# Helkafen/find-tfbs

Measured on AMD Instinct MI355X. Metric: haplotype-windows scored/sec, higher is better.
Workload: dtype fp4xfp6->f32 bound + int32 exact

## Files before the change

### find-tfbs_amd/csrc/ctx_assembly.hip

```cpp
#include "ctx.hpp"

using namespace tfbs;

AsmArgs tfbs::asm_args(tfbs_ctx *ctx, const Batch &B, int mode) {
    AsmArgs a{};
    a.haps = ctx->img.haps.p;
    a.druns = ctx->img.druns.p;
    a.regions = ctx->img.regions.p;
    a.hap_reuse = ctx->img.hap_reuse.p;
    a.region_asm = ctx->img.region_asm.p;
    a.inner = ctx->img.inner.p;
    a.mmeta = ctx->tabs.m_meta.p;
    a.slot_mfma = ctx->tabs.slot_mfma.p;
    a.any_dense = (!ctx->plan.fast_tiles.empty() || !ctx->plan.gen_tiles.empty() || !ctx->plan.di_tiles.empty()) ? 1 : 0;
    a.n_slots = B.n_slots;
    a.hpb = ctx->knobs.mfma_hpb;
    a.hitl = ctx->scan.hitl.p;
    a.hitn = ctx->scan.hitn.p;
    a.cand_cap = ctx->scan.scan_hit_cap;
    a.mfma = ctx->plan.m_supers.empty() ? 0 : 1;
    a.ref_hits = ctx->scan.ref_hits.p;
    a.ref_count = ctx->scan.ref_count.p;
    a.spill_sorted = ctx->scan.spill_sorted.p;
    a.spill_off = ctx->scan.spill_boff.p;
// ... 142 lines not shown
    uint64_t t_lo = UINT64_MAX, t_hi = 0;
    double busy = 0;
    for (uint32_t r = 0; r < nr; r++) {
        const uint64_t *p = &h[(size_t)r * kKfProfWords];
        if (!p[6]) continue;
        t_lo = std::min(t_lo, p[0]);
        t_hi = std::max(t_hi, p[6]);
        busy += (double)(p[6] - p[0]);
    }
    {
        std::vector<std::pair<std::pair<uint64_t, uint64_t>, uint32_t>> ev;
        for (uint32_t r = 0; r < nr; r++)
            if (h[(size_t)r * kKfProfWords + 6]) ev.push_back({{h[(size_t)r * kKfProfWords + 14], h[(size_t)r * kKfProfWords]}, r});
        std::sort(ev.begin(), ev.end());
        double gap = 0, late = 0, early_end = 0;
        uint32_t n_gap = 0, n_groups = 0;
        for (size_t i = 0; i < ev.size(); i++) {
            const uint64_t *p = &h[(size_t)ev[i].second * kKfProfWords];
            const bool first = i == 0 || ev[i - 1].first.first != ev[i].first.first;
            const bool last = i + 1 == ev.size() || ev[i + 1].first.first != ev[i].first.first;
            if (first) {
                n_groups++;
                late += (double)(p[0] - t_lo);
            } else {
                gap += (double)(p[0] - h[(size_t)ev[i - 1].second * kKfProfWords + 6]);
                n_gap++;
            }
            if (last) early_end += (double)(t_hi - p[6]);
        }
        if (n_groups)
            fprintf(stderr, "[kf prof] %u workgroups: mean gap between a workgroup's regions %.1f us (%u gaps), first "
                            "region start after the kernel's first %.1f us, last end before the kernel's last %.1f us\n",
                    n_groups, n_gap ? gap / n_gap / 100.0 : 0.0, n_gap, late / n_groups / 100.0, early_end / n_groups / 100.0);
    }
    uint32_t early = 0;
    for (uint32_t r = 0; r < nr; r++)
        if (h[(size_t)r * kKfProfWords + 6] && h[(size_t)r * kKfProfWords] < t_lo + 1000) early++;
    if (t_hi > t_lo)
        fprintf(stderr, "[kf prof] span %.1f us (first region start to last end, 100 MHz ticks), region-time %.1f us: "
                        "%.0f regions in flight on average; %u regions started in the first 10 us\n",
                (t_hi - t_lo) / 100.0, busy / 100.0, busy / (double)(t_hi - t_lo), early);
    const double d = n ? n : 1;
    fprintf(stderr,
            "[kf prof] front ticks/region: region record + reference hit list (round 1) %.0f, descriptors + hitn + "
            "first runs + meta (round 2) %.0f, hitn scan %.0f, runs staged %.0f, reference hits + barrier %.0f; in front of "
            "a region, ticket atomic to order entry %.0f\n",
            fr[0] / d, fr[1] / d, fr[2] / d, fr[3] / d, fr[4] / d, tkt / d);
    fprintf(stderr,
            "[kf prof] regions %u of %u ticks/region: descr+hitn %.0f refs %.0f dirty %.0f lists %.0f keys %.0f "
            "chunks %.0f (of which var-list atomics %.0f) (max total %.0f); per region: U %.1f entries %.1f dirty-refs %.1f corrections %.1f rows "
            "%.1f chunks %.2f in-LDS %.2f refs %.1f\n",
            n, nr, ph[0] / d, ph[1] / d, ph[2] / d, ph[3] / d, ph[4] / d, ph[5] / d, at / d, mx, sz[0] / d, sz[1] / d,
            sz[2] / d, sz[3] / d, sz[4] / d, sz[5] / d, sz[6] / d, sz[7] / d);
    return TFBS_OK;
}

int tfbs::assembly_wait(tfbs_ctx *ctx, Batch &B) {
    for (int round = 0; ctx->asmb.asm_state == 1; round++) {
        if (round == 8) return tfbs::fail(TFBS_E_NOMEM, "scan / key lists still full after 8 reruns");
        HIP_TRY(hipEventSynchronize(ctx->asmb.asm_ev));
        const uint32_t nspill = ctx->asmb.asm_host[kCtrOver], ncand = ctx->asmb.asm_host[kCtrOver + 1];
        const uint64_t *vt = reinterpret_cast<const uint64_t *>(ctx->asmb.asm_host.p + kCtrVarTot);
        const uint64_t nk = vt[0], nc = vt[1];
        if (ctx->knobs.debug_over && ctx->asmb.asm_host[kCtrRedoN]) {
            std::vector<uint32_t> redo(ctx->asmb.asm_host[kCtrRedoN]);
            HIP_TRY(hipMemcpy(redo.data(), ctx->asmb.asm_redo.p, redo.size() * 4, hipMemcpyDeviceToHost));
            uint64_t su = 0, sr = 0;
            uint32_t mu = 0, mi = 0;
            for (uint32_t r : redo) {
                const DevRegion &rg = B.regions[r];
                su += rg.hap_count;
                mu = std::max(mu, rg.hap_count);
                mi = std::max(mi, rg.n_inner);
                for (uint32_t l = 0; l < rg.hap_count; l++) sr += B.haps[rg.hap_begin + l].n_druns;
            }
            const uint32_t *why = ctx->asmb.asm_host.p + kCtrWhy;
            fprintf(stderr, "tfbs assembly: %zu regions left to key_asm: mean haplotypes %.1f (max %u), max inner %u, "
                            "mean diff runs %.1f; reasons: shape %u lists %u runs %u refs %u arena(cor) %u arena(cnt) %u\n",
                    redo.size(), (double)su / redo.size(), mu, mi, (double)sr / redo.size(), why[0], why[1], why[2],
                    why[3], why[4], why[5]);
        }
        if (ctx->knobs.debug_over)
            fprintf(stderr, "tfbs assembly: spill %u/%u candidates %u/%u left to key_asm %u arena %u/%u varying keys "
                            "%llu/%u counts %llu/%llu\n", nspill, ctx->scan.spill_cap, ncand, ctx->scan.cand_over_cap,
                    ctx->asmb.asm_host[kCtrRedoN], ctx->asmb.asm_host[kCtrCorUsed], ctx->asmb.cor_cap,
                    (unsigned long long)nk, ctx->asmb.var_keys_cap, (unsigned long long)nc,
                    (unsigned long long)ctx->asmb.var_cap);
        int rc;
        const bool need_post = !ctx->asmb.stages.post && (nspill || ncand);
        const bool need_wide = !ctx->asmb.stages.wide && ctx->asmb.asm_host[kCtrNeedWide], need_left = !ctx->asmb.stages.leftover && ctx->asmb.asm_host[kCtrRedoN];
        if (need_post || need_wide || need_left) {
            ctx->asmb.asm_full = true;
            ctx->asmb.asm_reruns++;
            ctx->asmb.asm_reruns_post += need_post ? 1 : 0;
            ctx->asmb.asm_post_rerun = need_post;
            ctx->asmb.asm_reruns_wide += need_wide ? 1 : 0;
            ctx->asmb.asm_reruns_left += need_left ? 1 : 0;
            rc = enqueue_assembly(ctx, B, true);
            ctx->asmb.asm_full = false;
            if (rc) return rc;
            continue;
        }
        if (ctx->asmb.asm_host[kCtrCorUsed] > ctx->asmb.cor_cap)
            ctx->asmb.cor_cap = (uint32_t)std::min<uint64_t>((uint64_t)ctx->asmb.asm_host[kCtrCorUsed] * 5 / 4, 1u << 30);
        if (nspill > ctx->scan.spill_cap || ncand > ctx->scan.cand_over_cap) {
            grow_cap(ctx->scan.spill_cap, ncand > ctx->scan.cand_over_cap ? 2 * std::max(nspill, 1024u) : nspill, UINT32_MAX / 4);
// ... 300 lines not shown
```

### find-tfbs_amd/csrc/key_kernels.hip

```cpp
#include <hip/hip_runtime.h>

#include <mutex>

#include <algorithm>
#include <cstdio>
#include <cstdlib>
#include <string>
#include <type_traits>

#include "keys.hpp"

namespace tfbs {
namespace {

constexpr int kAsmBlock = 256;
constexpr uint32_t kAsmWaves = kAsmBlock / 64;
constexpr uint32_t kAsmCounters = 6144;
constexpr uint32_t kAsmHaps = 1024;

constexpr uint32_t kAsmRuns = 2048;
constexpr uint32_t kAsmHits = 2048;
constexpr uint32_t kAsmRefs = 256;
constexpr uint32_t kAsmKeyWords = 2048;
constexpr uint32_t kAsmKeyWin = 32 * kAsmKeyWords;
// ... 391 lines not shown
using KfTyped = std::true_type;
using KfAny = std::false_type;
typedef uint32_t kf_u32x2 __attribute__((ext_vector_type(2)));
__device__ __forceinline__ uint32_t ld_global(const uint32_t *p) {
    return *(const __attribute__((address_space(1))) uint32_t *)p;
}
__device__ __forceinline__ uint2 ld_global(const uint2 *p) {
    const kf_u32x2 v = *(const __attribute__((address_space(1))) kf_u32x2 *)p;
    return make_uint2(v.x, v.y);
}
__device__ __forceinline__ void st_global(uint32_t *p, uint32_t v) {
    *(__attribute__((address_space(1))) uint32_t *)p = v;
}

__device__ __forceinline__ void arrived(uint32_t &x) { asm volatile("" : "+v"(x)); }

template <class Put>
__device__ __forceinline__ void wave_push(Put &&put, uint32_t *n, uint32_t cap, bool want, uint32_t v) {
    const uint64_t m = __ballot(want);
    if (!m) return;
    const uint32_t lane = threadIdx.x & 63, leader = (uint32_t)__builtin_ctzll(m);
    uint32_t base = 0;
    if (lane == leader) base = atomicAdd(n, (uint32_t)__popcll(m));
    base = (uint32_t)__shfl((int)base, (int)leader);
    if (want) {
        const uint32_t at = base + __builtin_amdgcn_mbcnt_hi((uint32_t)(m >> 32), __builtin_amdgcn_mbcnt_lo((uint32_t)m, 0));
        if (at < cap) put(at, v);
    }
}

template <uint32_t kFWaves>
__device__ __forceinline__ uint32_t block_excl_scan(uint32_t v, uint32_t *s_w, uint32_t &total) {
    const uint32_t lane = threadIdx.x & 63, wave = threadIdx.x >> 6;
    uint32_t x = v;
#pragma unroll
    for (int o = 1; o < 64; o <<= 1) {
        const uint32_t y = (uint32_t)__shfl_up((int)x, o);
        if (lane >= (uint32_t)o) x += y;
    }
    if (lane == 63) s_w[wave] = x;
    __syncthreads();
    uint32_t pre = 0, tot = 0;
#pragma unroll
    for (uint32_t w = 0; w < kFWaves; w++) {
        const uint32_t t = s_w[w];
        pre += w < wave ? t : 0u;
        tot += t;
    }
    __syncthreads();
    total = tot;
    return pre + x - v;
}

#ifndef TFBS_KF_WAVES
#define TFBS_KF_WAVES 1
#endif
template <class C>
__global__ __launch_bounds__(C::kBlock) __attribute__((amdgpu_waves_per_eu(C::kBlock == 1024 ? 1 : TFBS_KF_WAVES)))
void key_fast_kernel(AsmArgs A, uint32_t first, uint32_t count, uint32_t which) {
    constexpr int kFBlock = C::kBlock;
    constexpr uint32_t kFWaves = C::kWaves, kFHapLds = C::kHapLds, kFCor = C::kCor, kFRefs = C::kRefs,
                       kFCnt = C::kCnt, kFRuns = C::kRuns, kFRows = C::kRows, kFLists = C::kLists;
    constexpr uint32_t kPerW = kFKeyWords >= (uint32_t)kFBlock ? kFKeyWords / kFBlock : 1u;
    __shared__ uint32_t s_cor[kFCor];
    __shared__ uint4 s_ref[kFRefs];
    __shared__ uint32_t s_hap[kFHapLds];
    __shared__ uint32_t s_cnt[kFCnt];
    uint2 *const s_run = reinterpret_cast<uint2 *>(s_cnt);
    __shared__ uint32_t s_bits[kFKeyWords], s_rbase[kFKeyWords];
    __shared__ uint32_t s_rkey[kFRows], s_rr[kFRows];
    __shared__ uint32_t s_loff[kFLists + 1], s_lidx[kFLists];
    __shared__ uint32_t s_w[kFWaves];
    __shared__ uint32_t s_ncor, s_nref, s_nvar, s_arena, s_ndirty;
    __shared__ unsigned long long s_vbase, s_obase;
    const uint32_t tid = threadIdx.x, lane = tid & 63, wave = tid >> 6;
    auto process = [&](const uint32_t r, const uint32_t by_ticket, const uint64_t t_ticket) {
    auto stamp = [&](uint32_t k, uint64_t v) {
        if (A.prof && tid == 0) A.prof[kKfProfWords * (size_t)r + k] = v;
    };
    stamp(0, wall_clock64());
    stamp(20, t_ticket);
    uint32_t ft = tid;
    arrived(ft);
    const uint32_t *const none = reinterpret_cast<const uint32_t *>(A.regions + r);
    auto have = [&](bool c, const auto *p) { return c ? p : reinterpret_cast<decltype(p)>(none); };
    const bool spills = A.spill_count != nullptr;
    uint32_t n_rc = ld_global(have(A.mfma, A.ref_count + r));
    const uint2 rh = ld_global(have(A.mfma, reinterpret_cast<const uint2 *>(A.ref_hits) + (size_t)r * kRefPerRegion + (ft & 63u)));
    uint32_t rh_g = rh.x, rh_i = rh.y;
    uint32_t sp_n = ld_global(have(spills, A.spill_count));
    uint32_t sp_c = ld_global(have(spills, A.spill_cnt + r));
    uint32_t sp_o = ld_global(have(spills, A.spill_off + r));
    DevRegion rg = A.regions[r];
    uint4 ra = A.region_asm[r];
    arrived(n_rc), arrived(rh_g), arrived(rh_i), arrived(sp_n), arrived(sp_c), arrived(sp_o);
    arrived(rg.hap_count), arrived(ra.x);
    if (!spills) sp_n = 0;
    stamp(16, wall_clock64());
    const uint32_t U = rg.hap_count, n_inner = rg.n_inner, K = A.n_slots * n_inner;
    const uint64_t ko = (uint64_t)rg.inner_off * A.n_slots;
    uint32_t pw = TFBS_PATH_FAST | (kFBlock == 1024 ? TFBS_PATH_BIG : 0u) | by_ticket;
    auto trace = [&](uint32_t w) {
        if (A.path && tid == 0) A.path[r] = w;
    };
    if (U == 0 || K == 0) {
        trace(pw);
        for (uint32_t j = tid; j < K; j += kFBlock) {
            A.key_first[ko + j] = 0;
            A.key_flags[ko + j] = 0;
        }
        return;
    }
    auto give_up = [&](uint32_t why) {
        if (tid == 0) {
            A.redo[atomicAdd(A.redo_n, 1u)] = r;
            if (A.why) atomicAdd(A.why + why, 1u);
        }
        trace(pw | TFBS_PATH_GIVEUP | (why << TFBS_PATH_WHY_SHIFT));
    };
    if (U > (kFMaxU < A.fast_max_u ? kFMaxU : A.fast_max_u) || K > 32 * kFKeyWords || n_inner > 32) return give_up(0);
    const uint32_t hb = rg.hap_begin;
    const bool refs_on = A.mfma && rg.ref_hap != UINT32_MAX;
    const uint32_t run0 = (uint32_t)__builtin_amdgcn_readfirstlane((int)ra.x);
    const uint32_t nruns = (uint32_t)__builtin_amdgcn_readfirstlane((int)ra.y);
    const uint32_t lmax = (uint32_t)__builtin_amdgcn_readfirstlane((int)ra.z);
    if (tid == 0) s_ncor = s_nref = s_ndirty = 0;
    const uint32_t g_lo = hb / A.hpb, g_hi = (hb + U - 1) / A.hpb;
    const uint32_t nl = A.mfma ? (g_hi + 1 - g_lo) * kMBlockWaves : 0u;
    auto list_idx = [&](uint32_t t) -> uint32_t { return g_lo * kMBlockWaves + t; };
    const bool lists_staged = nl <= kFLists;
    if (!lists_staged) pw |= TFBS_PATH_LISTS_SLICED;
    if (nruns >= 65536) return give_up(2);
    if (nruns > kFRuns) pw |= TFBS_PATH_RUNS_L2;
    constexpr uint32_t kHapQ = kFHapLds / kFBlock;
// ... 36 lines not shown
    stamp(1, wall_clock64());
    auto hap_info = [&](uint32_t l) -> uint32_t {
        if (l < kFHapLds) return s_hap[l];
        return ld_global(A.hap_reuse + hb + l);
    };
    auto run_at = [&](auto typed, uint32_t k) -> uint2 {
        if constexpr (decltype(typed)::value) {
            return s_run[k];
        } else {
            if (runs_lds) return s_run[k];
            return ld_global(druns + k);
        }
    };
    if (runs_lds) {
        if (tid < nruns) s_run[tid] = make_uint2(run_a, run_b);
        for (uint32_t k = tid + kFBlock; k < nruns; k += kFBlock) s_run[k] = ld_global(druns + k);
    }
    stamp(18, wall_clock64());
    const uint2 sp = sp_n && sp_c ? make_uint2(sp_o, sp_o + sp_c) : make_uint2(0, 0);
    if (refs_on) {
        if (tid < n_list) {
            const uint32_t at = atomicAdd(&s_nref, 1u);
            if (at < kFRefs) s_ref[at] = make_ref_loaded(A, rg, m_len, m_depth, m_slot, rh_i);
        }
        for (uint32_t e = sp.x + tid; e < sp.y; e += kFBlock) {
            const uint32_t *q = A.spill_sorted + 3 * (size_t)e;
            if (q[0] >> 31) {
                const uint32_t at = atomicAdd(&s_nref, 1u);
                if (at < kFRefs) s_ref[at] = make_ref(A, rg, q[1], q[2]);
            }
        }
    }
    __syncthreads();
    const uint32_t nref = s_nref;
    stamp(19, wall_clock64());
    if (nref > kFRefs) return give_up(3);
    const bool pairwise = (uint64_t)U * nref <= 65536;
    if (!pairwise) pw |= TFBS_PATH_WALK;
    if (!pairwise) {
        uint4 mine = make_uint4(0, 0, 0, 0);
        uint32_t rank = 0;
        if (tid < nref) {
            mine = s_ref[tid];
            for (uint32_t j = 0; j < nref; j++) {
                const uint32_t w = s_ref[j].y;
                rank += (w < mine.y || (w == mine.y && j < tid)) ? 1u : 0u;
            }
        }
        __syncthreads();
        if (tid < nref) s_ref[rank] = mine;
        __syncthreads();
    }
    stamp(2, wall_clock64());
    auto dirty_masks = [&](auto typed, auto &&f) {
        for (uint32_t l0 = wave * 64; l0 < U; l0 += kFBlock) {
            const uint32_t l = l0 + lane;
            const uint32_t x = l < U ? hap_info(l) : kFNone;
            const uint32_t k0 = x == kFNone ? 0u : x & 0xFFFFu, k1 = x == kFNone ? 0u : k0 + (x >> 16);
            for (uint32_t p0 = 0; p0 < nref; p0 += 64) {
                const uint32_t np = min(64u, nref - p0);
                uint32_t rw = 0, re = 0;
                if (lane < np) {
                    const uint4 q = s_ref[p0 + lane];
                    rw = q.y;
                    re = q.y + (q.z & 0xFFFFu) - 1;
                }
                uint64_t m = 0;
                for (uint32_t i = 0; __ballot(i < k1 - k0) != 0; i++) {
                    uint2 ab = make_uint2(0xFFFFFFFFu, 0u);
                    if (i < k1 - k0) ab = run_at(typed, k0 + i);
                    for (uint32_t p = 0; p < np; p++) {
                        const uint32_t w = (uint32_t)__builtin_amdgcn_readlane((int)rw, (int)p);
                        const uint32_t e = (uint32_t)__builtin_amdgcn_readlane((int)re, (int)p);
                        if (ab.x <= e && ab.y >= w) m |= 1ull << p;
                    }
                }
                f(l, p0, m);
            }
        }
    };
    auto dirty_walk = [&](auto typed, auto &&f) {
        for (uint32_t l = tid; l < U; l += kFBlock) {
            const uint32_t x = hap_info(l);
            if (x == kFNone) continue;
            const uint32_t k0 = x & 0xFFFFu, k1 = k0 + (x >> 16);
            uint32_t p = 0;
            for (uint32_t k = k0; k < k1 && p < nref; k++) {
                const uint2 ab = run_at(typed, k);
                const uint32_t a = ab.x, b = ab.y;
                const uint32_t lo = a >= kMChunkCols * kMMaxChunks - 1 ? a - (kMChunkCols * kMMaxChunks - 1) : 0u;
                while (p < nref && s_ref[p].y < lo) p++;
                for (; p < nref && s_ref[p].y <= b; p++) {
                    const uint4 q = s_ref[p];
                    bool dirty = false;
                    for (uint32_t k2 = k0; k2 < k1 && !dirty; k2++) {
                        const uint2 r2 = run_at(typed, k2);
                        dirty = run_meets(r2.x, r2.y, q.y, q.z & 0xFFFFu);
                    }
                    if (dirty) f(l, q);
                }
            }
        }
    };
    auto slots = [&](uint32_t c, uint32_t *ctr) -> uint32_t {
        if (!__ballot(c > 1)) {
            const uint64_t m = __ballot(c != 0);
            if (!m) return 0;
            const uint32_t leader = (uint32_t)__builtin_ctzll(m);
            uint32_t base = 0;
            if (lane == leader) base = atomicAdd(ctr, (uint32_t)__popcll(m));
            return (uint32_t)__shfl((int)base, (int)leader) +
                   __builtin_amdgcn_mbcnt_hi((uint32_t)(m >> 32), __builtin_amdgcn_mbcnt_lo((uint32_t)m, 0));
        }
        uint32_t x = c;
#pragma unroll
        for (int o = 1; o < 64; o <<= 1) {
            const uint32_t y = (uint32_t)__shfl_up((int)x, o);
            if (lane >= (uint32_t)o) x += y;
        }
        const uint32_t tot = (uint32_t)__shfl((int)x, 63);
        uint32_t base = 0;
        if (lane == 0 && tot) base = atomicAdd(ctr, tot);
        return (uint32_t)__shfl((int)base, 0) + x - c;
    };
    auto list_mask = [&](uint32_t l, uint32_t p0, uint64_t m, uint32_t *ctr, auto &&put) -> uint32_t {
        uint32_t c = 0;
        for (uint64_t b = m; b; b &= b - 1) c += __popc(s_ref[p0 + (uint32_t)__builtin_ctzll(b)].w);
        uint32_t at = slots(c, ctr);
        for (uint64_t b = m; b; b &= b - 1) {
            const uint4 q = s_ref[p0 + (uint32_t)__builtin_ctzll(b)];
            for (uint32_t w = q.w; w; w &= w - 1, at++) put(at, cor_entry(q.x + __builtin_ctz(w), l, 1));
        }
        return c;
    };
    const uint32_t rpl = nref <= 1 ? 1u : nref >= 64 ? 64u : 1u << (32 - __clz(nref - 1));
    const uint32_t hpw = 64 / rpl, n_p = (nref + rpl - 1) / rpl;
    const bool stepbits = pairwise && (U + kFWaves * hpw - 1) / (kFWaves * hpw) * n_p <= 64;
    uint32_t nd = 0;
    if (nref) {
        auto count_and_list = [&](auto typed) {
            if (pairwise)
                dirty_masks(typed, [&](uint32_t l, uint32_t p0, uint64_t m) {
                    nd += list_mask(l, p0, m, &s_ndirty, [&](uint32_t at, uint32_t v) {
                        if (at < kFCor) s_cor[kFCor - 1 - at] = v;
                    });
                });
            else
                dirty_walk(typed, [&](uint32_t, const uint4 &q) { nd += __popc(q.w); });
        };
        if (runs_lds) count_and_list(KfTyped{});
        else count_and_list(KfAny{});
    }
    uint32_t nD = 0;
    (void)block_excl_scan<kFWaves>(nd, s_w, nD);
    const bool dirty_listed = pairwise && nD <= kFCor;
    const uint32_t need = n_ent + (sp.y - sp.x) + nD;
    const bool in_lds = need <= (kFCor < A.cor_lds ? kFCor : A.cor_lds);
    pw |= (stepbits ? TFBS_PATH_STEPBITS : 0u) | (dirty_listed ? TFBS_PATH_DIRTY_LISTED : 0u) |
          (in_lds ? 0u : TFBS_PATH_COR_ARENA);
    if (tid == 0) {
        s_arena = kFNone;
        if (!in_lds) {
            const uint32_t at = atomicAdd(A.cor_used, need);
            if (at <= A.cor_cap && need <= A.cor_cap - at) s_arena = at;
            if (dirty_listed) s_ncor = nD;
        }
    }
    __syncthreads();
    if (!in_lds && s_arena == kFNone) return give_up(4);
    stamp(3, wall_clock64());
    uint32_t *const cor_g = A.cor_arena + (in_lds ? 0u : s_arena);
    auto cor_ld = [&](auto typed, uint32_t e) -> uint32_t {
        if constexpr (decltype(typed)::value) {
            return s_cor[e];
        } else {
            if (in_lds) return s_cor[e];
            return ld_global(cor_g + e);
        }
    };
    auto cor_st = [&](auto typed, uint32_t e, uint32_t v) {
        if constexpr (decltype(typed)::value) {
            s_cor[e] = v;
        } else {
            if (in_lds) s_cor[e] = v;
            else st_global(cor_g + e, v);
        }
    };
    if (!in_lds && dirty_listed)
        for (uint32_t e = tid; e < nD; e += kFBlock) st_global(cor_g + e, s_cor[kFCor - 1 - e]);
    const uint32_t nw = (K + 31) / 32;
    uint32_t nA = 0, nB = 0, ncor = 0, T = 0;
    auto lists_and_rows = [&](auto typed) {
    auto put = [&](uint32_t at, uint32_t v) { cor_st(typed, at, v); };
    const uint2 *hitl = reinterpret_cast<const uint2 *>(A.hitl);
    for (uint32_t l0 = 0; l0 < nl; l0 += kFLists) {
        const uint32_t nlc = min(kFLists, nl - l0);
        uint32_t tot = n_ent;
        if (!lists_staged) {
            uint32_t lc = 0;
            if (tid < nlc) {
                const uint32_t idx = list_idx(l0 + tid);
                lc = A.hitn[idx];
                s_lidx[tid] = idx;
            }
            const uint32_t off = block_excl_scan<kFWaves>(lc, s_w, tot);
            if (tid < nlc) s_loff[tid] = off;
            if (tid == 0) s_loff[nlc] = tot;
            __syncthreads();
        }
        for (uint32_t e0 = 0; e0 < tot; e0 += kFBlock * kFBatch) {
            uint2 h[kFBatch];
#pragma unroll
            for (uint32_t q = 0; q < kFBatch; q++) {
                const uint32_t e = e0 + q * kFBlock + tid;
                h[q] = make_uint2(hb + U, 0);
                if (e < tot) {
                    uint32_t lo = 0, hi = nlc - 1;
                    while (lo < hi) {
                        const uint32_t mid = (lo + hi + 1) / 2;
                        if (s_loff[mid] <= e) lo = mid;
                        else hi = mid - 1;
                    }
                    const uint32_t idx = s_lidx[lo];
                    h[q] = hitl[(size_t)(idx / kMBlockWaves) * A.cand_cap +
                                (size_t)(idx % kMBlockWaves) * (A.cand_cap / kMBlockWaves) + (e - s_loff[lo])];
                }
            }
#pragma unroll
            for (uint32_t q = 0; q < kFBatch; q++)
                wave_push(put, &s_ncor, need, h[q].x - hb < U, cor_entry(h[q].y, h[q].x - hb, 0));
        }
        __syncthreads();
    }
    for (uint32_t e0 = sp.x; e0 < sp.y; e0 += kFBlock) {
        const uint32_t e = e0 + tid;
        bool want = false;
        uint32_t v = 0;
        if (e < sp.y) {
            const uint32_t *q = A.spill_sorted + 3 * (size_t)e;
            want = !(q[0] >> 31) && q[1] - hb < U;
            v = cor_entry(q[2], q[1] - hb, 0);
        }
        wave_push(put, &s_ncor, need, want, v);
    }
    if (!dirty_listed && nref) {
        auto put_in = [&](uint32_t at, uint32_t v) {
            if (at < need) cor_st(typed, at, v);
        };
        if (pairwise)
            dirty_masks(typed, [&](uint32_t l, uint32_t p0, uint64_t m) { (void)list_mask(l, p0, m, &s_ncor, put_in); });
        else
            dirty_walk(typed, [&](uint32_t l, const uint4 &q) {
                uint32_t at = atomicAdd(&s_ncor, (uint32_t)__popc(q.w));
                for (uint32_t m = q.w; m; m &= m - 1, at++) put_in(at, cor_entry(q.x + __builtin_ctz(m), l, 1));
            });
    }
    for (uint32_t w = tid; w < nw; w += kFBlock) s_bits[w] = 0;
    __syncthreads();
    stamp(4, wall_clock64());
    nA = s_ncor, nB = in_lds && dirty_listed ? nD : 0u, ncor = nA + nB;
    for (uint32_t e = tid; e < nA; e += kFBlock) {
        const uint32_t c = cor_ld(typed, e);
        if (!cor_neg(c)) atomicOr(&s_bits[cor_key(c) >> 5], 1u << (cor_key(c) & 31u));
    }
    if (tid < nref)
        for (uint32_t m = s_ref[tid].w; m; m &= m - 1) {
            const uint32_t key = s_ref[tid].x + __builtin_ctz(m);
            atomicOr(&s_bits[key >> 5], 1u << (key & 31u));
        }
    if (A.any_dense)
        for (uint32_t j = tid; j < K; j += kFBlock)
            if (!A.slot_mfma[j / n_inner]) atomicOr(&s_bits[j >> 5], 1u << (j & 31u));
    __syncthreads();
    {
        constexpr uint32_t per = kPerW;
        uint32_t mine = 0;
#pragma unroll
        for (uint32_t q = 0; q < per; q++) {
            const uint32_t w = tid * per + q;
            if (w < nw) mine += __popc(s_bits[w]);
        }
        uint32_t run = block_excl_scan<kFWaves>(mine, s_w, T);
#pragma unroll
        for (uint32_t q = 0; q < per; q++) {
            const uint32_t w = tid * per + q;
            if (w < nw) {
                s_rbase[w] = run;
                run += __popc(s_bits[w]);
            }
        }
    }
    };
    if (in_lds && runs_lds) lists_and_rows(KfTyped{});
    else lists_and_rows(KfAny{});
    stamp(5, wall_clock64());
    auto row_of = [&](uint32_t j) { return s_rbase[j >> 5] + __popc(s_bits[j >> 5] & ((1u << (j & 31)) - 1u)); };
    const bool half = 4 * (lmax + 64) < 65536 && A.cor_lds != 0;
    uint32_t rows_per = min((half ? 2 : 1) * kFCnt / U, kFRows);
    uint16_t *const cnt16 = reinterpret_cast<uint16_t *>(s_cnt);
    bool h16 = half, cnt_arena = false;
    uint32_t *cnt_g = A.cor_arena;
    if ((T + rows_per - 1) / rows_per > 32 || A.cor_lds == 0) {
        h16 = false;
        cnt_arena = true;
        pw |= TFBS_PATH_CNT_ARENA;
        rows_per = min(T, kFRows);
        if (tid == 0) {
            s_arena = kFNone;
            const uint32_t want = rows_per * U, at = atomicAdd(A.cor_used, want);
            if (at <= A.cor_cap && want <= A.cor_cap - at) s_arena = at;
        }
        __syncthreads();
        if (s_arena == kFNone) return give_up(5);
        cnt_g = A.cor_arena + s_arena;
    }
    pw |= (h16 ? 0u : TFBS_PATH_U32) | (U > kFHapLds ? TFBS_PATH_HAP_GLOBAL : 0u);
    for (uint32_t j = tid; j < K; j += kFBlock)
        if (!((s_bits[j >> 5] >> (j & 31)) & 1u)) {
            A.key_first[ko + j] = 0;
            A.key_flags[ko + j] = 0;
        }
    const uint64_t dense_base = A.dense_base ? A.haps[hb].count_off : 0;
    uint64_t t_atomics = 0;
    auto chunks = [&](auto typed) {
    constexpr bool kTyped = decltype(typed)::value;
    auto cor_top = [&](uint32_t e) -> uint32_t { return kFCor - nB + (e - nA); };
    auto cor_at = [&](uint32_t e) -> uint32_t {
        if constexpr (kTyped) return s_cor[e < nA ? e : cor_top(e)];
        else return e < nA ? cor_ld(typed, e) : s_cor[cor_top(e)];
    };
    auto cnt_set = [&](uint32_t x, uint32_t v) {
        if (kTyped || h16) cnt16[x] = (uint16_t)v;
        else if (cnt_arena) st_global(cnt_g + x, v);
        else s_cnt[x] = v;
    };
    auto cnt_add = [&](uint32_t x, uint32_t d) {
        if (kTyped || h16) atomicAdd(&s_cnt[x >> 1], d << (16 * (x & 1u)));
        else if (cnt_arena) atomicAdd(&cnt_g[x], d);
        else atomicAdd(&s_cnt[x], d);
    };
    auto count_at = [&](uint32_t x) -> uint32_t {
        if (kTyped || h16) return (uint32_t)cnt16[x];
        if (cnt_arena) return ld_global(cnt_g + x);
        return s_cnt[x];
    };
    for (uint32_t e = tid; e < ncor; e += kFBlock) {
        const uint32_t c = cor_at(e), v = (row_of(cor_key(c)) << 12) | (c & 4095u);
        if (e < nA) cor_st(typed, e, v);
        else s_cor[cor_top(e)] = v;
    }
    uint32_t dedup_bits = 0;
    for (uint32_t i = 0, l = lane; l < U; i++, l += 64)
        if (hap_info(l) != kFNone) dedup_bits |= 1u << i;
    for (uint32_t t0 = 0; t0 < T; t0 += rows_per) {
        const uint32_t nrow = min(rows_per, T - t0);
        __syncthreads();
        if (tid == 0) s_nvar = 0;
        {
            constexpr uint32_t per = kPerW;
#pragma unroll
            for (uint32_t q = 0; q < per; q++) {
                const uint32_t w = tid * per + q;
                if (w >= nw) continue;
                uint32_t t = s_rbase[w], b = s_bits[w];
                if (t >= t0 + nrow || t + __popc(b) <= t0) continue;
                for (; b; b &= b - 1, t++)
                    if (t - t0 < nrow) s_rkey[t - t0] = 32 * w + __builtin_ctz(b);
            }
        }
        for (uint32_t rr = tid; rr < nrow; rr += kFBlock) s_rr[rr] = 0;
        __syncthreads();
        if (tid < nref)
            for (uint32_t m = s_ref[tid].w; m; m &= m - 1) {
                const uint32_t t = row_of(s_ref[tid].x + __builtin_ctz(m)) - t0;
                if (t < nrow) atomicAdd(&s_rr[t], 1u);
            }
        __syncthreads();
        for (uint32_t rr = wave; rr < nrow; rr += kFWaves) {
            const uint32_t j = s_rkey[rr], R = s_rr[rr];
            const bool dense = A.any_dense && !A.slot_mfma[j / n_inner];
            for (uint32_t i = 0, l = lane; l < U; i++, l += 64) {
                const uint32_t v = dense ? A.counts[dense_base + (uint64_t)j * rg.count_stride + l]
                                         : ((dedup_bits >> i) & 1u ? R : 0u);
                cnt_set(rr * U + l, v);
            }
        }
        __syncthreads();
        for (uint32_t e = tid; e < ncor; e += kFBlock) {
            const uint32_t c = cor_at(e);
            const uint32_t t = cor_key(c) - t0;
            if (t < nrow) cnt_add(t * U + cor_hap(c), cor_neg(c) ? 0xFFFFFFFFu : 1u);
        }
        __syncthreads();
        for (uint32_t rr = wave; rr < nrow; rr += kFWaves) {
            const uint32_t c0 = count_at(rr * U);
            uint32_t any = 0, diff = 0;
            for (uint32_t l = lane; l < U; l += 64) {
                const uint32_t c = count_at(rr * U + l);
                any |= c;
                diff |= c ^ c0;
            }
            const bool a = __ballot(any != 0) != 0, v = __ballot(diff != 0) != 0;
            if (lane == 0) {
                const uint32_t j = s_rkey[rr];
                A.key_first[ko + j] = c0;
                A.key_flags[ko + j] = (uint8_t)((a ? KEY_ANY : 0) | (v ? KEY_VARIES : 0));
                s_rr[rr] = v ? atomicAdd(&s_nvar, 1u) : kFNone;
            }
        }
        __syncthreads();
        const uint64_t ta = A.prof ? wall_clock64() : 0;
        if (tid == 0 && s_nvar) {
            s_vbase = atomicAdd(A.var_tot, (unsigned long long)s_nvar);
            s_obase = atomicAdd(A.var_tot + 1, (unsigned long long)s_nvar * U);
        }
        __syncthreads();
        if (A.prof) t_atomics += wall_clock64() - ta;
        for (uint32_t rr = wave; rr < nrow; rr += kFWaves) {
            const uint32_t slot = s_rr[rr];
            if (slot == kFNone) continue;
            const uint64_t vi = s_vbase + slot, off = s_obase + (uint64_t)slot * U;
            if (vi >= A.var_keys_cap || off + U > A.var_cap) continue;
            if (lane == 0) A.var_keys[vi] = DevVarKey{r, s_rkey[rr], off};
            for (uint32_t l = lane; l < U; l += 64) A.var_counts[off + l] = count_at(rr * U + l);
        }
    }
    };
    if (in_lds && h16) chunks(KfTyped{});
    else chunks(KfAny{});
    stamp(6, wall_clock64());
    stamp(7, t_atomics);
    stamp(8, U);
    stamp(9, n_ent);
    stamp(10, nD);
    stamp(11, ncor);
    stamp(12, T);
    stamp(13, (T + rows_per - 1) / rows_per);
    stamp(14, blockIdx.x | (which << 24));
    stamp(15, nref);
    trace(pw);
    };
    __shared__ uint32_t s_tk;
    const bool tickets = A.persist && gridDim.x < count;
    uint32_t i = blockIdx.x;
    while (i < count) {
        uint32_t tk = 0;
        uint64_t t_ticket = A.prof ? wall_clock64() : 0;
        if (tickets && tid == 0) tk = gridDim.x + atomicAdd(A.next + which, 1u);
        const uint32_t r = A.order ? A.order[first + i] : first + i;
        if (A.prof) {
            asm volatile("" ::"v"(r));
            t_ticket = wall_clock64() - t_ticket;
        }
        process(r, i == blockIdx.x ? 0u : (uint32_t)TFBS_PATH_TICKET, t_ticket);
        if (!tickets) break;
        if (tid == 0) s_tk = tk;
        __syncthreads();
        i = s_tk;
        __syncthreads();
    }
    if (A.report_fast && blockIdx.x == 0 && tid < 2) A.report[tid] = A.report_src ? A.report_src[tid] : 0u;
}

__global__ __launch_bounds__(256) void spill_hist_kernel(const uint32_t *__restrict__ over, uint32_t cap,
                                                          const uint32_t *__restrict__ spill, uint32_t *__restrict__ bcnt) {
    const uint32_t n = min(over[0], cap);
    for (uint32_t e = blockIdx.x * 256 + threadIdx.x; e < n; e += gridDim.x * 256)
        atomicAdd(&bcnt[spill[3 * (size_t)e] & 0x7FFFFFFFu], 1u);
}

__global__ __launch_bounds__(1024) void spill_scan_kernel(const uint32_t *__restrict__ over, uint32_t *__restrict__ bcnt,
                                                          uint32_t n, uint32_t *__restrict__ boff) {
    __shared__ uint32_t s[1024];
    if (over[0] == 0) return;
    uint32_t carry = 0;
    for (uint32_t b0 = 0; b0 < n; b0 += 1024) {
        const uint32_t i = b0 + threadIdx.x;
        const uint32_t v = i < n ? bcnt[i] : 0;
        s[threadIdx.x] = v;
        __syncthreads();
        for (uint32_t o = 1; o < 1024; o <<= 1) {
            const uint32_t t = threadIdx.x >= o ? s[threadIdx.x - o] : 0;
            __syncthreads();
            s[threadIdx.x] += t;
// ... 422 lines not shown
```

### find-tfbs_amd/csrc/keys.hpp

```cpp
#pragma once

#include <hip/hip_runtime.h>

#include <algorithm>
#include <cstddef>
#include <cstdint>

#include "batch.hpp"
#include "scan.hpp"

namespace tfbs {

struct AsmArgs {
    const DevHap *haps;
    const uint32_t *druns;
    const DevRegion *regions;
    const uint32_t *hap_reuse;
    const uint4 *region_asm;
    const int32_t *inner;
    const int32_t *mmeta;
    const uint8_t *slot_mfma;
    uint32_t any_dense;
    uint32_t n_slots;
    uint32_t hpb;
    const uint32_t *hitl, *hitn;
    uint32_t cand_cap;
    uint32_t mfma;
    const uint32_t *ref_hits, *ref_count;
    const uint32_t *spill_sorted, *spill_off, *spill_cnt;
    const uint32_t *spill_count;
    uint32_t spill_cap;
    uint32_t *counts;
    uint32_t dense_base;
    uint32_t *scratch;
    int mode;
    uint32_t *key_first;
    uint8_t *key_flags;
    DevVarKey *var_keys;
    uint32_t var_keys_cap;
    uint32_t *var_counts;
    uint64_t var_cap;
    unsigned long long *var_tot;
    uint32_t *redo, *redo_n;
    uint32_t fast_max_u;
    uint32_t *cor_arena;
    uint32_t cor_cap;
    uint32_t *cor_used;
    uint32_t cor_lds;
    uint32_t *why;
    const uint32_t *report_src;
    uint32_t *report;
    uint32_t report_fast;
    const uint32_t *order;
    uint32_t persist;
    uint32_t *next;
    uint64_t *prof;
    uint32_t *path;
    uint32_t grid_cap;
};

constexpr uint32_t kKfProfWords = 24;

enum AsmCtr : uint32_t {
    kCtrOver = 0,
    kCtrRedoN = 2,
    kCtrCorUsed = 3,
    kCtrVarTot = 4,
    kCtrWhy = 8,
    kCtrNext = 16,
    kCtrWgDone = 18,
    kCtrNeedWide = 20,
    kCtrPostDone = 21,
    kAsmCtrWords = 24,
};
inline size_t asm_bucket_words(uint32_t nr) { return 2 * ((size_t)std::max<uint32_t>(1, nr) + 1); }

int launch_key_asm(const AsmArgs &a, uint32_t n_regions, hipStream_t stream);
int launch_key_fast(const AsmArgs &a, uint32_t n_regions, uint32_t n_big, hipStream_t stream, hipStream_t side,
                    hipEvent_t fork, hipEvent_t join, bool leftover = true);
uint32_t key_fast_big_u();
int launch_asm_report(const uint32_t *over, uint32_t *ctr, hipStream_t stream);
uint32_t key_asm_lds_counters();
int launch_spill_buckets(const uint32_t *over, uint32_t cap, const uint32_t *spill, uint32_t n_regions, uint32_t *bcnt,
                         uint32_t *boff, uint32_t *sorted, hipStream_t stream, bool bcnt_zeroed = false);
int launch_pair_table(const uint64_t *rows, uint32_t n_regions, uint32_t n_samples, uint32_t *pab, uint32_t *pcnt,
                      uint32_t *pair_n, uint16_t *pidx, hipStream_t stream);
int launch_memb_fill(const uint32_t *meta, const uint32_t *ids, const uint16_t *loc, uint32_t n_rows, uint32_t Hp,
                     uint16_t *memb, hipStream_t stream);
int launch_key_encode(const uint32_t *var_counts, const DevVarKey *keys, uint32_t n_keys, const uint32_t *pab,
                      const uint32_t *pcnt, const uint32_t *pair_n, const uint16_t *pidx, uint32_t region0,
                      uint32_t n_samples, EncHdr *hdr, uint32_t *vals, uint32_t *hist, uint8_t *codes,
                      hipStream_t stream);
int launch_val_compact(const uint32_t *vals, const uint32_t *hist, uint32_t n_keys, const uint32_t *off, uint32_t *ov,
                       uint32_t *oh, hipStream_t stream);
int launch_code_compact(const uint8_t *codes, uint32_t n_keys, uint32_t n_samples, const uint64_t *off, uint8_t *dst,
                        hipStream_t stream);

}
```

Baseline: 331700 billion.

## Restructure key_fast dirty-hit listing and chunk loop; raise waves per EU

Replaces the per-hap dirty mask loop with a grouped readlane comparison that splits references across spare waves and lists hits with one atomic per block of 64 haps. For non-1024-thread blocks, rewrites the chunk loop so each wave owns rows with one row per lane: row keys are built once when they fit, reference counts come from ballots, classification and variable-key slot allocation are done per lane, and the var_tot atomics are issued by the first two threads. It also raises the default waves-per-EU hint from 1 to 4 and adds optional fine-grained profiling compiled in only under a macro. The changes trade simpler code and register headroom for more parallel work per region, and they add an extra barrier.

```diff
diff --git a/find-tfbs_amd/csrc/ctx_assembly.hip b/find-tfbs_amd/csrc/ctx_assembly.hip
--- a/find-tfbs_amd/csrc/ctx_assembly.hip
+++ b/find-tfbs_amd/csrc/ctx_assembly.hip
@@ -218,6 +218,18 @@
             "%.1f chunks %.2f in-LDS %.2f refs %.1f\n",
             n, nr, ph[0] / d, ph[1] / d, ph[2] / d, ph[3] / d, ph[4] / d, ph[5] / d, at / d, mx, sz[0] / d, sz[1] / d,
             sz[2] / d, sz[3] / d, sz[4] / d, sz[5] / d, sz[6] / d, sz[7] / d);
+    double fine[kKfProfFineN] = {}, fine_sum = 0;
+    for (uint32_t r = 0; r < nr; r++) {
+        const uint64_t *p = &h[(size_t)r * kKfProfWords];
+        if (!p[6]) continue;
+        for (uint32_t k = 0; k < kKfProfFineN; k++) fine[k] += (double)p[kKfProfFine + k], fine_sum += (double)p[kKfProfFine + k];
+    }
+    if (fine_sum != 0)
+        fprintf(stderr,
+                "[kf prof] fine ticks/region: dirty: pair loop %.0f listing %.0f scan %.0f; chunks: remap %.0f row keys + R "
+                "%.0f base fill %.0f corrections %.0f classification %.0f var atomics %.0f varying rows %.0f\n",
+                fine[0] / d, fine[1] / d, fine[2] / d, fine[3] / d, fine[4] / d, fine[5] / d, fine[6] / d, fine[7] / d,
+                fine[8] / d, fine[9] / d);
     return TFBS_OK;
 }
 
diff --git a/find-tfbs_amd/csrc/key_kernels.hip b/find-tfbs_amd/csrc/key_kernels.hip
--- a/find-tfbs_amd/csrc/key_kernels.hip
+++ b/find-tfbs_amd/csrc/key_kernels.hip
@@ -467,8 +467,13 @@
     return pre + x - v;
 }
 
+#ifdef TFBS_KF_FINE
+#define KF_FINE(...) __VA_ARGS__
+#else
+#define KF_FINE(...)
+#endif
 #ifndef TFBS_KF_WAVES
-#define TFBS_KF_WAVES 1
+#define TFBS_KF_WAVES 4
 #endif
 template <class C>
 __global__ __launch_bounds__(C::kBlock) __attribute__((amdgpu_waves_per_eu(C::kBlock == 1024 ? 1 : TFBS_KF_WAVES)))
@@ -487,7 +492,7 @@
     __shared__ uint32_t s_loff[kFLists + 1], s_lidx[kFLists];
     __shared__ uint32_t s_w[kFWaves];
     __shared__ uint32_t s_ncor, s_nref, s_nvar, s_arena, s_ndirty;
-    __shared__ unsigned long long s_vbase, s_obase;
+    __shared__ unsigned long long s_vb[2];
     const uint32_t tid = threadIdx.x, lane = tid & 63, wave = tid >> 6;
     auto process = [&](const uint32_t r, const uint32_t by_ticket, const uint64_t t_ticket) {
     auto stamp = [&](uint32_t k, uint64_t v) {
@@ -495,6 +500,13 @@
     };
     stamp(0, wall_clock64());
     stamp(20, t_ticket);
+    KF_FINE(uint64_t tf[kKfProfFineN] = {}; uint64_t tf_last = 0;
+            auto fine_start = [&]() { tf_last = wall_clock64(); };
+            auto fine = [&](uint32_t k) {
+                const uint64_t t = wall_clock64();
+                tf[k] += t - tf_last;
+                tf_last = t;
+            };)
     uint32_t ft = tid;
     arrived(ft);
     const uint32_t *const none = reinterpret_cast<const uint32_t *>(A.regions + r);
@@ -637,32 +649,73 @@
         __syncthreads();
     }
     stamp(2, wall_clock64());
-    auto dirty_masks = [&](auto typed, auto &&f) {
-        for (uint32_t l0 = wave * 64; l0 < U; l0 += kFBlock) {
+    KF_FINE(fine_start();)
+    constexpr uint32_t kDGroup = 8;
+    const uint32_t wv = (uint32_t)__builtin_amdgcn_readfirstlane((int)wave);
+    const uint32_t nblk = (U + 63) / 64;
+    const uint32_t shares = 2 * nblk <= kFWaves ? kFWaves / nblk : 1u;
+    auto dirty_hits = [&](auto typed, uint32_t *ctr, auto &&put) -> uint32_t {
+        uint32_t total = 0;
+        const uint32_t share = shares > 1 ? wv / nblk : 0u;
+        if (share >= shares) return 0;
+        const uint32_t per = (nref + shares - 1) / shares;
+        const uint32_t h0 = min(share * per, nref), h1 = min(h0 + per, nref);
+        for (uint32_t l0 = 64 * (shares > 1 ? wv % nblk : wv); l0 < U; l0 += shares > 1 ? 64 * nblk : kFBlock) {
             const uint32_t l = l0 + lane;
             const uint32_t x = l < U ? hap_info(l) : kFNone;
-            const uint32_t k0 = x == kFNone ? 0u : x & 0xFFFFu, k1 = x == kFNone ? 0u : k0 + (x >> 16);
-            for (uint32_t p0 = 0; p0 < nref; p0 += 64) {
-                const uint32_t np = min(64u, nref - p0);
-                uint32_t rw = 0, re = 0;
+            const uint32_t k0 = x == kFNone ? 0u : x & 0xFFFFu, nk = x == kFNone ? 0u : x >> 16;
+            for (uint32_t p0 = h0; p0 < h1; p0 += 64) {
+                const uint32_t np = min(64u, h1 - p0);
+                uint32_t rw = 0xFFFFFFFFu, re = 0, rx = 0, rb = 0;
                 if (lane < np) {
                     const uint4 q = s_ref[p0 + lane];
-                    rw = q.y;
-                    re = q.y + (q.z & 0xFFFFu) - 1;
+                    rw = q.y, re = q.y + (q.z & 0xFFFFu) - 1, rx = q.x, rb = q.w;
                 }
-                uint64_t m = 0;
-                for (uint32_t i = 0; __ballot(i < k1 - k0) != 0; i++) {
-                    uint2 ab = make_uint2(0xFFFFFFFFu, 0u);
-                    if (i < k1 - k0) ab = run_at(typed, k0 + i);
-                    for (uint32_t p = 0; p < np; p++) {
-                        const uint32_t w = (uint32_t)__builtin_amdgcn_readlane((int)rw, (int)p);
-                        const uint32_t e = (uint32_t)__builtin_amdgcn_readlane((int)re, (int)p);
-                        if (ab.x <= e && ab.y >= w) m |= 1ull << p;
+                uint32_t mlo = 0, mhi = 0, tot = 0;
+                for (uint32_t g0 = 0; g0 < np; g0 += kDGroup) {
+                    uint32_t w[kDGroup], e[kDGroup];
+                    uint64_t mk[kDGroup];
+#pragma unroll
+                    for (uint32_t g = 0; g < kDGroup; g++) {
+                        w[g] = (uint32_t)__builtin_amdgcn_readlane((int)rw, (int)(g0 + g));
+                        e[g] = (uint32_t)__builtin_amdgcn_readlane((int)re, (int)(g0 + g));
+                        mk[g] = 0;
+                    }
+                    for (uint32_t i = 0; __ballot(i < nk) != 0; i++) {
+                        uint2 ab = make_uint2(0xFFFFFFFFu, 0u);
+                        if (i < nk) ab = run_at(typed, k0 + i);
+#pragma unroll
+                        for (uint32_t g = 0; g < kDGroup; g++)
+                            mk[g] |= __builtin_amdgcn_uicmp(ab.x, e[g], 37) & __builtin_amdgcn_uicmp(ab.y, w[g], 35);
+                    }
+#pragma unroll
+                    for (uint32_t g = 0; g < kDGroup; g++) {
+                        if (lane == g0 + g) mlo = (uint32_t)mk[g], mhi = (uint32_t)(mk[g] >> 32);
+                        tot += (uint32_t)__popcll(mk[g]) * (uint32_t)__popc((uint32_t)__builtin_amdgcn_readlane((int)rb, (int)(g0 + g)));
                     }
                 }
-                f(l, p0, m);
-            }
-        }
+                KF_FINE(fine(0);)
+                if (tot == 0) continue;
+                uint32_t base = 0;
+                if (lane == 0) base = atomicAdd(ctr, tot);
+                base = (uint32_t)__builtin_amdgcn_readfirstlane((int)base);
+                total += tot;
+                for (uint64_t hm = __ballot((mlo | mhi) != 0); hm; hm &= hm - 1) {
+                    const int p = __builtin_ctzll(hm);
+                    const uint32_t lo = (uint32_t)__builtin_amdgcn_readlane((int)mlo, p);
+                    const uint32_t hi = (uint32_t)__builtin_amdgcn_readlane((int)mhi, p);
+                    const uint32_t qx = (uint32_t)__builtin_amdgcn_readlane((int)rx, p);
+                    const uint32_t qb = (uint32_t)__builtin_amdgcn_readlane((int)rb, p);
+                    const bool mine = (((uint64_t)hi << 32 | lo) >> lane) & 1u;
+                    const uint32_t rank = __builtin_amdgcn_mbcnt_hi(hi, __builtin_amdgcn_mbcnt_lo(lo, 0));
+                    const uint32_t n = (uint32_t)__popc(lo) + (uint32_t)__popc(hi);
+                    for (uint32_t b = qb; b; b &= b - 1, base += n)
+                        if (mine) put(base + rank, cor_entry(qx + (uint32_t)__builtin_ctz(b), l, 1));
+                }
+                KF_FINE(fine(1);)
+            }
+        }
+        return total;
     };
     auto dirty_walk = [&](auto typed, auto &&f) {
         for (uint32_t l = tid; l < U; l += kFBlock) {
@@ -687,50 +740,18 @@
             }
         }
     };
-    auto slots = [&](uint32_t c, uint32_t *ctr) -> uint32_t {
-        if (!__ballot(c > 1)) {
-            const uint64_t m = __ballot(c != 0);
-            if (!m) return 0;
-            const uint32_t leader = (uint32_t)__builtin_ctzll(m);
-            uint32_t base = 0;
-            if (lane == leader) base = atomicAdd(ctr, (uint32_t)__popcll(m));
-            return (uint32_t)__shfl((int)base, (int)leader) +
-                   __builtin_amdgcn_mbcnt_hi((uint32_t)(m >> 32), __builtin_amdgcn_mbcnt_lo((uint32_t)m, 0));
-        }
-        uint32_t x = c;
-#pragma unroll
-        for (int o = 1; o < 64; o <<= 1) {
-            const uint32_t y = (uint32_t)__shfl_up((int)x, o);
-            if (lane >= (uint32_t)o) x += y;
-        }
-        const uint32_t tot = (uint32_t)__shfl((int)x, 63);
-        uint32_t base = 0;
-        if (lane == 0 && tot) base = atomicAdd(ctr, tot);
-        return (uint32_t)__shfl((int)base, 0) + x - c;
-    };
-    auto list_mask = [&](uint32_t l, uint32_t p0, uint64_t m, uint32_t *ctr, auto &&put) -> uint32_t {
-        uint32_t c = 0;
-        for (uint64_t b = m; b; b &= b - 1) c += __popc(s_ref[p0 + (uint32_t)__builtin_ctzll(b)].w);
-        uint32_t at = slots(c, ctr);
-        for (uint64_t b = m; b; b &= b - 1) {
-            const uint4 q = s_ref[p0 + (uint32_t)__builtin_ctzll(b)];
-            for (uint32_t w = q.w; w; w &= w - 1, at++) put(at, cor_entry(q.x + __builtin_ctz(w), l, 1));
-        }
-        return c;
-    };
     const uint32_t rpl = nref <= 1 ? 1u : nref >= 64 ? 64u : 1u << (32 - __clz(nref - 1));
     const uint32_t hpw = 64 / rpl, n_p = (nref + rpl - 1) / rpl;
     const bool stepbits = pairwise && (U + kFWaves * hpw - 1) / (kFWaves * hpw) * n_p <= 64;
     uint32_t nd = 0;
     if (nref) {
         auto count_and_list = [&](auto typed) {
-            if (pairwise)
-                dirty_masks(typed, [&](uint32_t l, uint32_t p0, uint64_t m) {
-                    nd += list_mask(l, p0, m, &s_ndirty, [&](uint32_t at, uint32_t v) {
-                        if (at < kFCor) s_cor[kFCor - 1 - at] = v;
-                    });
+            if (pairwise) {
+                const uint32_t c = dirty_hits(typed, &s_ndirty, [&](uint32_t at, uint32_t v) {
+                    if (at < kFCor) s_cor[kFCor - 1 - at] = v;
                 });
-            else
+                nd += lane == 0 ? c : 0u;
+            } else
                 dirty_walk(typed, [&](uint32_t, const uint4 &q) { nd += __popc(q.w); });
         };
         if (runs_lds) count_and_list(KfTyped{});
@@ -754,6 +775,7 @@
     __syncthreads();
     if (!in_lds && s_arena == kFNone) return give_up(4);
     stamp(3, wall_clock64());
+    KF_FINE(fine(2);)
     uint32_t *const cor_g = A.cor_arena + (in_lds ? 0u : s_arena);
     auto cor_ld = [&](auto typed, uint32_t e) -> uint32_t {
         if constexpr (decltype(typed)::value) {
@@ -829,11 +851,12 @@
         wave_push(put, &s_ncor, need, want, v);
     }
     if (!dirty_listed && nref) {
+        KF_FINE(fine_start();)
         auto put_in = [&](uint32_t at, uint32_t v) {
             if (at < need) cor_st(typed, at, v);
         };
         if (pairwise)
-            dirty_masks(typed, [&](uint32_t l, uint32_t p0, uint64_t m) { (void)list_mask(l, p0, m, &s_ncor, put_in); });
+            (void)dirty_hits(typed, &s_ncor, put_in);
         else
             dirty_walk(typed, [&](uint32_t l, const uint4 &q) {
                 uint32_t at = atomicAdd(&s_ncor, (uint32_t)__popc(q.w));
@@ -878,6 +901,7 @@
     };
     if (in_lds && runs_lds) lists_and_rows(KfTyped{});
     else lists_and_rows(KfAny{});
+    __syncthreads();
     stamp(5, wall_clock64());
     auto row_of = [&](uint32_t j) { return s_rbase[j >> 5] + __popc(s_bits[j >> 5] & ((1u << (j & 31)) - 1u)); };
     const bool half = 4 * (lmax + 64) < 65536 && A.cor_lds != 0;
@@ -929,30 +953,48 @@
         if (cnt_arena) return ld_global(cnt_g + x);
         return s_cnt[x];
     };
+    KF_FINE(fine_start();)
     for (uint32_t e = tid; e < ncor; e += kFBlock) {
         const uint32_t c = cor_at(e), v = (row_of(cor_key(c)) << 12) | (c & 4095u);
         if (e < nA) cor_st(typed, e, v);
         else s_cor[cor_top(e)] = v;
     }
+    KF_FINE(fine(3);)
     uint32_t dedup_bits = 0;
     for (uint32_t i = 0, l = lane; l < U; i++, l += 64)
         if (hap_info(l) != kFNone) dedup_bits |= 1u << i;
+    auto ref_count = [&](uint32_t j, uint32_t fx, uint32_t fw) -> uint32_t {
+        uint32_t d = j - fx;
+        uint32_t R = (uint32_t)__popcll(__ballot(d < 32 && ((fw >> d) & 1u)));
+        for (uint32_t p0 = 64; p0 < nref; p0 += 64) {
+            uint32_t x = 0, w = 0;
+            if (p0 + lane < nref) {
+                const uint4 q = s_ref[p0 + lane];
+                x = q.x, w = q.w;
+            }
+            d = j - x;
+            R += (uint32_t)__popcll(__ballot(d < 32 && ((w >> d) & 1u)));
+        }
+        return R;
+    };
+    auto row_keys = [&](uint32_t t0, uint32_t nrow) {
+        constexpr uint32_t per = kPerW;
+#pragma unroll
+        for (uint32_t q = 0; q < per; q++) {
+            const uint32_t w = tid * per + q;
+            if (w >= nw) continue;
+            uint32_t t = s_rbase[w], b = s_bits[w];
+            if (t >= t0 + nrow || t + __popc(b) <= t0) continue;
+            for (; b; b &= b - 1, t++)
+                if (t - t0 < nrow) s_rkey[t - t0] = 32 * w + __builtin_ctz(b);
+        }
+    };
+    if constexpr (kFBlock == 1024) {
     for (uint32_t t0 = 0; t0 < T; t0 += rows_per) {
         const uint32_t nrow = min(rows_per, T - t0);
         __syncthreads();
         if (tid == 0) s_nvar = 0;
-        {
-            constexpr uint32_t per = kPerW;
-#pragma unroll
-            for (uint32_t q = 0; q < per; q++) {
-                const uint32_t w = tid * per + q;
-                if (w >= nw) continue;
-                uint32_t t = s_rbase[w], b = s_bits[w];
-                if (t >= t0 + nrow || t + __popc(b) <= t0) continue;
-                for (; b; b &= b - 1, t++)
-                    if (t - t0 < nrow) s_rkey[t - t0] = 32 * w + __builtin_ctz(b);
-            }
-        }
+        row_keys(t0, nrow);
         for (uint32_t rr = tid; rr < nrow; rr += kFBlock) s_rr[rr] = 0;
         __syncthreads();
         if (tid < nref)
@@ -996,25 +1038,138 @@
         __syncthreads();
         const uint64_t ta = A.prof ? wall_clock64() : 0;
         if (tid == 0 && s_nvar) {
-            s_vbase = atomicAdd(A.var_tot, (unsigned long long)s_nvar);
-            s_obase = atomicAdd(A.var_tot + 1, (unsigned long long)s_nvar * U);
+            s_vb[0] = atomicAdd(A.var_tot, (unsigned long long)s_nvar);
+            s_vb[1] = atomicAdd(A.var_tot + 1, (unsigned long long)s_nvar * U);
         }
         __syncthreads();
         if (A.prof) t_atomics += wall_clock64() - ta;
         for (uint32_t rr = wave; rr < nrow; rr += kFWaves) {
             const uint32_t slot = s_rr[rr];
             if (slot == kFNone) continue;
-            const uint64_t vi = s_vbase + slot, off = s_obase + (uint64_t)slot * U;
+            const uint64_t vi = s_vb[0] + slot, off = s_vb[1] + (uint64_t)slot * U;
             if (vi >= A.var_keys_cap || off + U > A.var_cap) continue;
             if (lane == 0) A.var_keys[vi] = DevVarKey{r, s_rkey[rr], off};
             for (uint32_t l = lane; l < U; l += 64) A.var_counts[off + l] = count_at(rr * U + l);
         }
+    }
+    } else {
+    const bool keys_once = T <= kFRows;
+    uint32_t ct = tid;
+    arrived(ct);
+    const uint32_t cl = ct & 63u;
+    if (keys_once) row_keys(0, T);
+    static_assert(kFRows <= 64 * kFWaves, "a wave's rows of a chunk: one per lane");
+    for (uint32_t t0 = 0; t0 < T; t0 += rows_per) {
+        const uint32_t nrow = min(rows_per, T - t0);
+        __syncthreads();
+        if (!keys_once) {
+            row_keys(t0, nrow);
+            __syncthreads();
+        }
+        const uint32_t kb = keys_once ? t0 : 0u;
+        KF_FINE(fine(4);)
+        uint32_t fx = 0, fw = 0;
+        if (lane < nref) {
+            const uint4 q = s_ref[lane];
+            fx = q.x, fw = q.w;
+        }
+        const uint32_t my_rr = wv + cl * kFWaves;
+        const uint32_t my_j = s_rkey[kb + min(my_rr, nrow - 1)];
+        for (uint32_t rr = wv, ri = 0; rr < nrow; rr += kFWaves, ri++) {
+            const uint32_t j = (uint32_t)__builtin_amdgcn_readlane((int)my_j, (int)ri);
+            const uint32_t R = ref_count(j, fx, fw);
+            const bool dense = A.any_dense && !A.slot_mfma[j / n_inner];
+            for (uint32_t i = 0, l = lane; l < U; i++, l += 64) {
+                const uint32_t v = dense ? A.counts[dense_base + (uint64_t)j * rg.count_stride + l]
+                                         : ((dedup_bits >> i) & 1u ? R : 0u);
+                cnt_set(rr * U + l, v);
+            }
+        }
+        __syncthreads();
+        KF_FINE(fine(5);)
+        for (uint32_t e = tid; e < ncor; e += kFBlock) {
+            const uint32_t c = cor_at(e);
+            const uint32_t t = cor_key(c) - t0;
+            if (t < nrow) cnt_add(t * U + cor_hap(c), cor_neg(c) ? 0xFFFFFFFFu : 1u);
+        }
+        __syncthreads();
+        KF_FINE(fine(6);)
+        uint32_t my_res = 0;
+        {
+            const uint32_t la = min(cl, U - 1), lb = min(cl + 64, U - 1);
+            uint32_t na = count_at(min(wv, nrow - 1) * U + la), nb = count_at(min(wv, nrow - 1) * U + lb);
+            for (uint32_t rr = wv, i = 0; rr < nrow; rr += kFWaves, i++) {
+                const uint32_t ca = na, cb = nb, nx = min(rr + kFWaves, nrow - 1) * U;
+                na = count_at(nx + la), nb = count_at(nx + lb);
+                const uint32_t c0 = (uint32_t)__builtin_amdgcn_readfirstlane((int)ca);
+                uint32_t any = ca | cb, diff = (ca ^ c0) | (cb ^ c0);
+                for (uint32_t l = cl + 128; l < U; l += 64) {
+                    const uint32_t c = count_at(rr * U + l);
+                    any |= c;
+                    diff |= c ^ c0;
+                }
+                const bool a = __ballot(any != 0) != 0, v = __ballot(diff != 0) != 0;
+                if (cl == i) my_res = c0 | ((a ? KEY_ANY : 0u) | (v ? KEY_VARIES : 0u)) << 30;
+            }
+        }
+        if (my_rr < nrow) s_rr[my_rr] = my_res >> 30;
+        __syncthreads();
+        KF_FINE(fine(7);)
+        const uint64_t ta = A.prof ? wall_clock64() : 0;
+        uint32_t slot = 0, nvar = 0;
+        for (uint32_t r0 = 0; r0 < nrow; r0 += 64) {
+            const uint64_t m = __ballot(r0 + cl < nrow && (s_rr[min(r0 + cl, nrow - 1)] & KEY_VARIES));
+            if ((my_rr >> 6) == (r0 >> 6)) slot = nvar + (uint32_t)__popcll(m & ((1ull << (my_rr & 63u)) - 1ull));
+            nvar += (uint32_t)__popcll(m);
+        }
+        unsigned long long got = 0;
+        if (nvar && ct < 2) got = atomicAdd(A.var_tot + ct, ct ? (unsigned long long)nvar * U : (unsigned long long)nvar);
+        if (my_rr < nrow) {
+            A.key_first[ko + my_j] = my_res & 0x3FFFFFFFu;
+            A.key_flags[ko + my_j] = (uint8_t)(my_res >> 30);
+        }
+        if (nvar == 0) continue;
+        if (ct < 2) s_vb[ct] = got;
+        __syncthreads();
+        KF_FINE(fine(8);)
+        if (A.prof) t_atomics += wall_clock64() - ta;
+        auto uni64 = [](unsigned long long v) -> uint64_t {
+            return (uint64_t)(uint32_t)__builtin_amdgcn_readfirstlane((int)(uint32_t)v) |
+                   (uint64_t)(uint32_t)__builtin_amdgcn_readfirstlane((int)(uint32_t)(v >> 32)) << 32;
+        };
+        const uint64_t vbase = uni64(s_vb[0]), obase = uni64(s_vb[1]);
+        const uint64_t my_off = obase + (uint64_t)slot * U;
+        const bool my_put = my_rr < nrow && ((my_res >> 30) & KEY_VARIES) && vbase + slot < A.var_keys_cap &&
+                            my_off + U <= A.var_cap;
+        if (my_put) A.var_keys[vbase + slot] = DevVarKey{r, my_j, my_off};
+        uint64_t vm = __ballot(my_put);
+        if (vm) {
+            const uint32_t la = min(cl, U - 1), lb = min(cl + 64, U - 1);
+            uint32_t nx = (wv + (uint32_t)__builtin_ctzll(vm) * kFWaves) * U;
+            uint32_t na = count_at(nx + la), nb = count_at(nx + lb);
+            while (vm) {
+                const int i = __builtin_ctzll(vm);
+                vm &= vm - 1;
+                const uint32_t ca = na, cb = nb, x0 = nx;
+                if (vm) {
+                    nx = (wv + (uint32_t)__builtin_ctzll(vm) * kFWaves) * U;
+                    na = count_at(nx + la), nb = count_at(nx + lb);
+                }
+                const uint64_t off = obase + (uint64_t)(uint32_t)__builtin_amdgcn_readlane((int)slot, i) * U;
+                if (cl < U) A.var_counts[off + cl] = ca;
+                if (cl + 64 < U) A.var_counts[off + cl + 64] = cb;
+                for (uint32_t l = cl + 128; l < U; l += 64) A.var_counts[off + l] = count_at(x0 + l);
+            }
+        }
+        KF_FINE(fine(9);)
+    }
     }
     };
     if (in_lds && h16) chunks(KfTyped{});
     else chunks(KfAny{});
     stamp(6, wall_clock64());
     stamp(7, t_atomics);
+    KF_FINE(for (uint32_t k = 0; k < kKfProfFineN; k++) stamp(kKfProfFine + k, tf[k]);)
     stamp(8, U);
     stamp(9, n_ent);
     stamp(10, nD);
diff --git a/find-tfbs_amd/csrc/keys.hpp b/find-tfbs_amd/csrc/keys.hpp
--- a/find-tfbs_amd/csrc/keys.hpp
+++ b/find-tfbs_amd/csrc/keys.hpp
@@ -59,7 +59,8 @@
     uint32_t grid_cap;
 };
 
-constexpr uint32_t kKfProfWords = 24;
+constexpr uint32_t kKfProfWords = 40;
+constexpr uint32_t kKfProfFine = 24, kKfProfFineN = 10;
 
 enum AsmCtr : uint32_t {
     kCtrOver = 0,
```

Result: faster. 370100 billion (median of 6 runs) (+11.6%).
